# gudgud96/MR-MT3

Measured on AMD Instinct MI355X. Metric: train segments/sec (T5-small MT3Net, 256-frame mel, 1024-token target; log-mel + fwd + bwd + AdamW), higher is better.
Workload: dtype bf16; 1 GPU; BASELINE configs[1]: t5 bf16, 64 segments/GPU/step of 32768 samples @16kHz -> 256x512 mel, 1024-token targets, dropout 0.1 on, golden-recipe weights; segments_per_gpu=64, global_segments=64, parallelism=dp1

## Files before the change

include/mrmt3_hip.h:

```cpp
#ifndef MRMT3_HIP_H
#define MRMT3_HIP_H

#include <stddef.h>
#include <stdint.h>

#ifdef __cplusplus
extern "C" {
#endif

#define MRMT3_OK 0
#define MRMT3_ERR_INVALID_ARG 1
#define MRMT3_ERR_HIP 2
#define MRMT3_ERR_UNSUPPORTED 3
#define MRMT3_ERR_COMM 4

#define MRMT3_F32 0
#define MRMT3_BF16 1

int mrmt3_version(void);
const char* mrmt3_last_error(void);
void* mrmt3_host_alloc(size_t bytes);
void mrmt3_host_free(void* p);

#define MRMT3_CNT_GEMM_NT_TILE 0
// ... 167 lines not shown
                     int32_t* step_dev, float beta1, float beta2, float eps, float weight_decay,
                     float grad_scale, void* shadow_bf16, void* stream);
size_t mrmt3_grad_norm_workspace_elems(void);
int mrmt3_grad_norm(const float* g, size_t n, float grad_scale, float max_norm, int skip_nonfinite, float* ws,
                    size_t ws_elems, float* stat_dev, int32_t* skipped_dev, void* stream);
int mrmt3_adamw_step_clipped(float* p, const float* g, float* m, float* v, size_t n, const float* lr_dev,
                             int32_t* step_dev, float beta1, float beta2, float eps, float weight_decay,
                             float grad_scale, const float* stat_dev, float clip_value, void* shadow_bf16,
                             void* stream);
int mrmt3_counter_add(int32_t* ctr, int32_t delta, void* stream);
int mrmt3_transpose(const void* in, int in_dtype, void* out, int out_dtype, int rows, int cols,
                    void* stream);
int mrmt3_cast(const void* in, int in_dtype, void* out, int out_dtype, size_t n, void* stream);
int mrmt3_transpose_batched(const void* src_bf16, void* dst_bf16, const void* desc_table,
                            const int* tile_start, int n_mats, int total_tiles, void* stream);

typedef struct mrmt3_decoder mrmt3_decoder;
typedef struct {
  const void* embed;
  const float* pos;
  const void* lm_head;
  const float* final_ln;
  const float* const* ln_self;
  const void* const* w_qkv;
  const void* const* w_o_self;
  const float* const* ln_cross;
  const void* const* w_q_cross;
  const void* const* w_o_cross;
  const float* const* ln_ff;
  const void* const* w_wi;
// ... 52 lines not shown
```

mr-mt3_amd/csrc/api.hip:

```cpp
#include <stdarg.h>
#include <stdio.h>
#include <stdlib.h>

#include <atomic>
#include <mutex>

#include "common.h"

static thread_local char g_err[512] = "";

void mrmt3_set_error(const char* fmt, ...) {
  va_list ap;
  va_start(ap, fmt);
  vsnprintf(g_err, sizeof(g_err), fmt, ap);
  va_end(ap);
}

#ifdef MRMT3_DIAG
int mrmt3_diag_env(const char* name) {
  const char* e = getenv(name);
  const int v = e ? atoi(e) : 0;
  if (v != 0) {
    static std::atomic<unsigned> warned{0};
    const unsigned bit = 1u << ((unsigned char)name[6] & 31);
// ... 57 lines not shown
    strcpy(g_knob_over[g_knob_n_over++].name, name);
  }
  g_knob_over[i].value = value;
  for (MrKnob* k = g_knob_sites; k != nullptr; k = k->next)
    if (strcmp(k->name, name) == 0) __atomic_store_n(&k->state, 0, __ATOMIC_RELEASE);
  return MRMT3_OK;
}

extern "C" int mrmt3_reset_knobs(void) {
  std::lock_guard<std::mutex> lock(g_knob_mu);
  g_knob_n_over = 0;
  for (MrKnob* k = g_knob_sites; k != nullptr; k = k->next) __atomic_store_n(&k->state, 0, __ATOMIC_RELEASE);
  return MRMT3_OK;
}

extern "C" int mrmt3_version(void) { return 117;  }
extern "C" const char* mrmt3_last_error(void) { return g_err; }

int mrmt3_cu_count() {
  static int n = 0;
  if (n == 0) {
    int dev = 0;
    hipDeviceProp_t prop;
    if (hipGetDevice(&dev) == hipSuccess && hipGetDeviceProperties(&prop, dev) == hipSuccess) n = prop.multiProcessorCount;
    if (n <= 0) n = 256;
  }
  return n;
}

extern "C" void* mrmt3_host_alloc(size_t bytes) {
  void* p = nullptr;
// ... 118 lines not shown
```

mr-mt3_amd/csrc/rowops.hip:

```cpp
#include "common.h"

#pragma clang fp contract(off)

template <typename T> __device__ __forceinline__ void load4(const T* p, float v[4]);
template <> __device__ __forceinline__ void load4<float>(const float* p, float v[4]) {
  f32x4 t = *(const f32x4*)p;
  v[0] = t.x; v[1] = t.y; v[2] = t.z; v[3] = t.w;
}
template <> __device__ __forceinline__ void load4<bf16_t>(const bf16_t* p, float v[4]) {
  u32x2 t = *(const u32x2*)p;
  v[0] = __uint_as_float(t.x << 16); v[1] = __uint_as_float(t.x & 0xFFFF0000u);
  v[2] = __uint_as_float(t.y << 16); v[3] = __uint_as_float(t.y & 0xFFFF0000u);
}
template <typename T> __device__ __forceinline__ void store4(T* p, const float v[4]);
template <> __device__ __forceinline__ void store4<float>(float* p, const float v[4]) {
  *(f32x4*)p = f32x4{v[0], v[1], v[2], v[3]};
}
template <> __device__ __forceinline__ void store4<bf16_t>(bf16_t* p, const float v[4]) {
  *(u32x2*)p = u32x2{pack_bf2(v[0], v[1]), pack_bf2(v[2], v[3])};
}

template <typename T> __device__ __forceinline__ void load4_nt(const T* p, float v[4]);
template <> __device__ __forceinline__ void load4_nt<float>(const float* p, float v[4]) {
  const f32x4 t = __builtin_nontemporal_load((const f32x4*)p);
// ... 965 lines not shown
  for (int i = 0; i < TLP_REGS; ++i) se += expf(v[i] - mx);
  se = wave_sum(se);
  if (lane == 0) out[row] = (lp[t] - mx) - logf(se);
}

extern "C" int mrmt3_token_logprob(const float* logits, const int64_t* targets, float* out, int rows, int V,
                                   int ignore_index, void* stream) {
  MR_CHECK_ARG(logits && targets && out && rows > 0 && V > 0, "token_logprob: bad args");
  MR_CHECK_ARG(V <= 64 * TLP_REGS, "token_logprob: vocab %d exceeds the %d logits a wave keeps in registers", V, 64 * TLP_REGS);
  const dim3 grid((unsigned)ceil_div(rows, 4)), block(256);
  hipLaunchKernelGGL(token_logprob_kernel, grid, block, 0, (hipStream_t)stream, logits, targets, out, rows, V, ignore_index);
  MR_CHECK_LAUNCH("token_logprob");
  return MRMT3_OK;
}

__global__ void adamw_kernel(float* __restrict__ p, const float* __restrict__ g, float* __restrict__ m,
                             float* __restrict__ v, size_t n4, const float* __restrict__ lr_dev,
                             const int32_t* __restrict__ step_dev, float b1, float b2, float eps, float wd,
                             float gscale, bf16_t* __restrict__ shadow) {
  const float lr = lr_dev[0];
  const int step = step_dev[0] + 1;
  const double bc1 = 1.0 - pow((double)b1, (double)step);
  const double bc2 = 1.0 - pow((double)b2, (double)step);
  const float step_size = (float)((double)lr / bc1);
  const float bc2_sqrt = (float)sqrt(bc2);
  const float decay = 1.f - lr * wd;
  for (size_t i = (size_t)blockIdx.x * blockDim.x + threadIdx.x; i < n4; i += (size_t)gridDim.x * blockDim.x) {
    float pv[4], gv[4], mv[4], vv[4];
    load4<float>(p + i * 4, pv);
    load4<float>(g + i * 4, gv);
    load4<float>(m + i * 4, mv);
    load4<float>(v + i * 4, vv);
#pragma unroll
    for (int e = 0; e < 4; ++e) {
      const float gr = gv[e] * gscale;
      pv[e] *= decay;
      mv[e] = mv[e] + (gr - mv[e]) * (1.f - b1);
      vv[e] = vv[e] * b2 + (1.f - b2) * gr * gr;
      const float denom = sqrtf(vv[e]) / bc2_sqrt + eps;
      pv[e] -= step_size * (mv[e] / denom);
    }
    store4<float>(p + i * 4, pv);
    store4<float>(m + i * 4, mv);
    store4<float>(v + i * 4, vv);
    if (shadow) store4<bf16_t>(shadow + i * 4, pv);
  }
}
__global__ void step_inc_kernel(int32_t* step) { step[0] += 1; }

extern "C" int mrmt3_adamw_step(float* p, const float* g, float* m, float* v, size_t n, const float* lr_dev,
                                int32_t* step_dev, float beta1, float beta2, float eps, float weight_decay,
                                float grad_scale, void* shadow_bf16, void* stream) {
  MR_CHECK_ARG(p && g && m && v && lr_dev && step_dev && n % 4 == 0, "adamw_step: bad args");
  hipStream_t s = (hipStream_t)stream;
  hipLaunchKernelGGL(adamw_kernel, dim3(ew_blocks(n / 4)), dim3(256), 0, s, p, g, m, v, n / 4, lr_dev, step_dev,
                     beta1, beta2, eps, weight_decay, grad_scale, (bf16_t*)shadow_bf16);
  MR_CHECK_LAUNCH("adamw_step");
  hipLaunchKernelGGL(step_inc_kernel, dim3(1), dim3(1), 0, s, step_dev);
  MR_CHECK_LAUNCH("adamw_step inc");
  return MRMT3_OK;
}
// ... 85 lines not shown
  hipLaunchKernelGGL(grad_sumsq_kernel, dim3(GN_BLOCKS), dim3(256), 0, s, g, n / 4, (double*)ws);
  MR_CHECK_LAUNCH("grad_norm");
  hipLaunchKernelGGL(grad_norm_finish_kernel, dim3(1), dim3(256), 0, s, (const double*)ws, grad_scale, max_norm,
                     skip_nonfinite, stat_dev, skipped_dev);
  MR_CHECK_LAUNCH("grad_norm finish");
  return MRMT3_OK;
}

__global__ void adamw_clipped_kernel(float* __restrict__ p, const float* __restrict__ g, float* __restrict__ m,
                                     float* __restrict__ v, size_t n4, const float* __restrict__ lr_dev,
                                     const int32_t* __restrict__ step_dev, float b1, float b2, float eps, float wd,
                                     float gscale, const float* __restrict__ stat, float clip_value,
                                     bf16_t* __restrict__ shadow) {
  if (stat[2] != 0.f) return;
  const float coef = stat[1];
  const float lr = lr_dev[0];
  const int step = step_dev[0] + 1;
  const double bc1 = 1.0 - pow((double)b1, (double)step);
  const double bc2 = 1.0 - pow((double)b2, (double)step);
  const float step_size = (float)((double)lr / bc1);
  const float bc2_sqrt = (float)sqrt(bc2);
  const float decay = 1.f - lr * wd;
  for (size_t i = (size_t)blockIdx.x * blockDim.x + threadIdx.x; i < n4; i += (size_t)gridDim.x * blockDim.x) {
    float pv[4], gv[4], mv[4], vv[4];
    load4<float>(p + i * 4, pv);
    load4<float>(g + i * 4, gv);
    load4<float>(m + i * 4, mv);
    load4<float>(v + i * 4, vv);
#pragma unroll
    for (int e = 0; e < 4; ++e) {
      float gr = gv[e] * gscale * coef;
      if (clip_value > 0.f) gr = gr > clip_value ? clip_value : (gr < -clip_value ? -clip_value : gr);
      pv[e] *= decay;
      mv[e] = mv[e] + (gr - mv[e]) * (1.f - b1);
      vv[e] = vv[e] * b2 + (1.f - b2) * gr * gr;
      const float denom = sqrtf(vv[e]) / bc2_sqrt + eps;
      pv[e] -= step_size * (mv[e] / denom);
    }
    store4<float>(p + i * 4, pv);
    store4<float>(m + i * 4, mv);
    store4<float>(v + i * 4, vv);
    if (shadow) store4<bf16_t>(shadow + i * 4, pv);
  }
}

extern "C" int mrmt3_adamw_step_clipped(float* p, const float* g, float* m, float* v, size_t n, const float* lr_dev,
                                        int32_t* step_dev, float beta1, float beta2, float eps, float weight_decay,
                                        float grad_scale, const float* stat_dev, float clip_value, void* shadow_bf16,
                                        void* stream) {
  MR_CHECK_ARG(p && g && m && v && lr_dev && step_dev && stat_dev && n % 4 == 0, "adamw_step_clipped: bad args");
  MR_CHECK_ARG(clip_value >= 0.f, "adamw_step_clipped: clip_value = %g is negative (0: no clamp)", (double)clip_value);
  hipStream_t s = (hipStream_t)stream;
  hipLaunchKernelGGL(adamw_clipped_kernel, dim3(ew_blocks(n / 4)), dim3(256), 0, s, p, g, m, v, n / 4, lr_dev, step_dev,
                     beta1, beta2, eps, weight_decay, grad_scale, stat_dev, clip_value, (bf16_t*)shadow_bf16);
  MR_CHECK_LAUNCH("adamw_step_clipped");
  hipLaunchKernelGGL(step_inc_kernel, dim3(1), dim3(1), 0, s, step_dev);
  MR_CHECK_LAUNCH("adamw_step_clipped inc");
  return MRMT3_OK;
// ... 122 lines not shown
      if (r < d.rows) q[0] = v0;
      if (r + 1 < d.rows) q[1] = v1;
    }
  }
}

extern "C" int mrmt3_transpose_batched(const void* src_bf16, void* dst_bf16, const void* desc_table,
                                       const int* tile_start, int n_mats, int total_tiles, void* stream) {
  MR_CHECK_ARG(src_bf16 && dst_bf16 && desc_table && tile_start && n_mats > 0 && total_tiles > 0, "transpose_batched: bad args");
  hipLaunchKernelGGL(transpose_batched_kernel, dim3((unsigned)total_tiles), dim3(256), 0, (hipStream_t)stream,
                     (const bf16_t*)src_bf16, (bf16_t*)dst_bf16, (const TrDesc*)desc_table, tile_start, n_mats);
  MR_CHECK_LAUNCH("transpose_batched");
  return MRMT3_OK;
}

extern "C" int mrmt3_transpose(const void* in, int in_dtype, void* out, int out_dtype, int rows, int cols,
                               void* stream) {
  MR_CHECK_ARG(in && out && rows > 0 && cols > 0, "transpose: bad args");
  dim3 grid((unsigned)ceil_div(cols, 32), (unsigned)ceil_div(rows, 32)), block(256);
  hipStream_t s = (hipStream_t)stream;
  if (in_dtype == MRMT3_F32 && out_dtype == MRMT3_BF16)
    hipLaunchKernelGGL((transpose_kernel<float, bf16_t>), grid, block, 0, s, (const float*)in, (bf16_t*)out, rows, cols);
  else if (in_dtype == MRMT3_F32 && out_dtype == MRMT3_F32)
    hipLaunchKernelGGL((transpose_kernel<float, float>), grid, block, 0, s, (const float*)in, (float*)out, rows, cols);
  else if (in_dtype == MRMT3_BF16 && out_dtype == MRMT3_BF16)
    hipLaunchKernelGGL((transpose_kernel<bf16_t, bf16_t>), grid, block, 0, s, (const bf16_t*)in, (bf16_t*)out, rows, cols);
  else
    hipLaunchKernelGGL((transpose_kernel<bf16_t, float>), grid, block, 0, s, (const bf16_t*)in, (float*)out, rows, cols);
  MR_CHECK_LAUNCH("transpose");
  return MRMT3_OK;
// ... 2 lines not shown
```

mr-mt3_amd/mrmt3/engine.py:

```python
from __future__ import annotations

import os

import torch

from . import lib
from .params import FlatParams
from .synthetic import sinusoid_table


class Tape:

    def __init__(self):
        self.ops = []

    def push(self, **kw):
        self.ops.append(kw)

    def pop(self):
        return self.ops.pop()


class Engine:
    def __init__(self, cfg: dict, flat: FlatParams, variant: str = "t5", segmem_length: int = 64,
# ... 7 lines not shown
        self.eps = cfg["layer_norm_epsilon"]
        self.max_pos = max_pos
        self._pos = None
        self._stream_ctr = 0
        self.seed = 365
        self.step_dev = None
        self.y_dtype = compute_dtype
        self.overlap_wgrad = False
        self.res_grad_dtype = (torch.bfloat16 if compute_dtype == torch.bfloat16 and
                               os.environ.get("MRMT3_RES_GRAD", "bf16") == "bf16" else torch.float32)
        self.head_dtype = "bf16"
        self._wt32 = {}
        self.lo_sites = os.environ.get("MRMT3_ATTN_LO", "all")
        self.norm_dw = lib.NormDwBatch() if os.environ.get("MRMT3_NORM_DW_BATCH", "1") != "0" else None
        self.tn_group = lib.TnGroup() if os.environ.get("MRMT3_TN_GROUP", "1") != "0" else None
        self.fuse_rows = int(os.environ.get("MRMT3_FUSE_ROWS", "6")) if compute_dtype == torch.bfloat16 else 0
        self.fuse_normbwd_max_k = int(os.environ.get("MRMT3_FUSE_NORMBWD_MAXK", "1152"))

    def pos(self, device):
        if self._pos is None or self._pos.device != device:
            self._pos = sinusoid_table(self.max_pos, self.d).to(device).contiguous()
        return self._pos

    def _sid(self):
        self._stream_ctr += 1
        return self._stream_ctr

    def W(self, name):
        return self.flat.W(name, self.dt)

    def ln(self, key):
        return self.flat.master(key)

    def WT(self, name):
        if self.dt == torch.bfloat16:
            return self.flat.WT(name)
        t = self._wt32.get(name)
        if t is None:
            w = self.flat.W(name, torch.float32)
            t = torch.empty(w.shape[1], w.shape[0], device=w.device, dtype=torch.float32)
            lib.transpose(w, t)
            self._wt32[name] = t
        return t

    def wgrad(self, a, b, out):
        if a.dtype == torch.float32:
            return lib.gemm_tn_f32(a, b, out, accumulate=True)
        if self.tn_group is not None and self.tn_group.ok(a, b, out):
            return self.tn_group.add(a, b, out, accumulate=True)
        return lib.gemm_tn(a, b, out, accumulate=True)

    def _norm_bwd(self, *a, **kw):
        if self.dt == torch.bfloat16:
            return lib.add_rmsnorm_bwd(*a, defer=self.norm_dw, **kw)
        want_dy = kw.pop("want_dy", True)
        dx1, _ = lib.add_rmsnorm_bwd(*a, defer=self.norm_dw, want_dy=False, **kw)
        if not want_dy:
            return dx1, None
        p = kw.get("p", 0.0)
        if p <= 0.0:
            return dx1, dx1
        return dx1, lib.dropmask_cast(dx1, p=p, seed=kw.get("seed", 0), stream_id=kw.get("stream_y", 0),
                                      step=kw.get("step"), out_dtype=torch.float32)

# ... 359 lines not shown
        head_f32 = self.head_dtype == "f32" and tape is None and self.dt == torch.bfloat16
        dec = self.stack_fwd("decoder", x, B, Lx, cfg["num_decoder_layers"], True, enc=enc_cat, Le=Lc, p=p, tape=tape,
                             out_dtype=torch.float32 if head_f32 else None, pack=pack)
        if variant == "segmem_v1":
            dec = dec.view(B, Lx, d)[:, Ls:].contiguous().view(B * Ld, d)
        if tape is not None:
            tape.push(kind="head", dec=dec)
        if not want_logits:
            return dec, tape
        w_head = f.W("lm_head", torch.float32) if head_f32 else self.W("lm_head")
        logits = lib.gemm_nt(dec, w_head, out_dtype=torch.float32)
        if pack is not None:
            return logits, tape
        return logits.view(B, Ld, self.V), tape

    def backward(self, tape, dlogits, on_layer_done=None):
        f, cfg, d = self.flat, self.cfg, self.d
        variant, Ls = self.variant, self.segmem_length
        t = tape.pop()
        assert t["kind"] == "head"
        dl = dlogits.reshape(-1, self.V)
        if dl.dtype != self.dt:
            dl = self._act(dl)
        self.wgrad(dl, t["dec"], f.GW("lm_head"))
        d_dec = lib.gemm_nt(dl, self.WT("lm_head"), out_dtype=torch.float32)
        if on_layer_done is not None:
            on_layer_done("lm_head", 0)
        din = next(o for o in reversed(tape.ops) if o["kind"] == "dec_in")
        B, Le, Ld, Lx, Lc, Ls = din["B"], din["Le"], din["Ld"], din["Lx"], din["Lc"], din["Ls"]
        variant = din["variant"]
        if variant == "segmem_v1":
            full = torch.zeros(B, Lx, d, device=d_dec.device, dtype=torch.float32)
            full[:, Ls:] = d_dec.view(B, Ld, d)
# ... 36 lines not shown
```

mr-mt3_amd/mrmt3/lib.py:

```python
from __future__ import annotations

import ctypes as C
import os
import re
import subprocess

import torch

F32, BF16 = 0, 1
_HERE = os.path.dirname(os.path.abspath(__file__))
LIB_PATH = os.environ.get("MRMT3_TOOL_LIB") or os.path.join(_HERE, "libmrmt3_hip.so")
HEADER_PATH = os.path.join(os.path.dirname(os.path.dirname(_HERE)), "include", "mrmt3_hip.h")
CSRC_DIR = os.path.join(os.path.dirname(_HERE), "csrc")
_lib = None

vp = C.c_void_p


def _header_text(path: str) -> str:
    return re.sub(r"/\*.*?\*/", "", open(path).read(), flags=re.S)


def header_symbols(path: str = HEADER_PATH):
    return sorted(set(re.findall(r"\b(mrmt3_[a-z0-9_]+)\s*\(", _header_text(path))))
# ... 56 lines not shown
            "(no CPU fallback). Run `python __graft_entry__.py` / `make -C mr-mt3_amd/csrc` first.")
    lib = C.CDLL(LIB_PATH)
    for name, (res, args) in _SIGS.items():
        if os.environ.get("MRMT3_TOOL_LIB") and not hasattr(lib, name):
            continue
        fn = getattr(lib, name)
        fn.restype = res
        fn.argtypes = args
    if not os.environ.get("MRMT3_TOOL_LIB") and lib.mrmt3_version() < MIN_VERSION:
        raise RuntimeError(f"{LIB_PATH} is version {lib.mrmt3_version()}, this binding needs >= {MIN_VERSION}: "
                           "a stale build — run `make -C mr-mt3_amd/csrc`")
    _lib = lib
    return lib


MIN_VERSION = 117
COUNTER_NAMES = ("gemm_nt_tile", "gemm_nt8", "gemm_nt_geglu", "tn_group", "tn8", "tn_tile", "attn_fwd", "attn_bwd",
                 "attn_bwd_onepass", "attn_f32", "tn_f32", "gemm_nt_splitk", "gemm_nt_addnorm", "gemm_nt_normbwd",
                 "gemm_nt_geglubwd", "attn_fwd_varlen", "attn_bwd_varlen")


def set_knob(name: str, value: int):
    _check(load().mrmt3_set_knob(name.encode(), int(value)), "set_knob")


def reset_knobs():
    _check(load().mrmt3_reset_knobs(), "reset_knobs")


def dispatch_counts(reset: bool = False) -> dict:
    arr = (C.c_ulonglong * len(COUNTER_NAMES))()
# ... 787 lines not shown
    return out


def cast(src, out):
    _dev(src, out)
    _check(load().mrmt3_cast(_p(src), _dt(src), _p(out), _dt(out), src.numel(), _stream()), "cast")
    return out


def transpose_batched(src_flat, dst_flat, desc_table, tile_start, n_mats, total_tiles):
    _dev(src_flat, dst_flat, desc_table, tile_start)
    _check(load().mrmt3_transpose_batched(_p(src_flat), _p(dst_flat), _p(desc_table), _p(tile_start), n_mats,
                                          total_tiles, _stream()), "transpose_batched")


COMM_ID_BYTES = 128


class Comm:

    def __init__(self, uid: bytes, rank: int, world: int):
        assert len(uid) == COMM_ID_BYTES
        self.rank, self.world = rank, world
        self._h = vp()
        buf = C.create_string_buffer(uid, COMM_ID_BYTES)
        _check(load().mrmt3_comm_create(buf, rank, world, C.byref(self._h)), "comm_create")
        import weakref
        self._fin = weakref.finalize(self, Comm._destroy, self._h)

    @staticmethod
# ... 92 lines not shown
```

mr-mt3_amd/mrmt3/params.py:

```python
from __future__ import annotations

from collections import OrderedDict

import torch

from . import lib
from .synthetic import state_dict_shapes


class FlatParams:
    def __init__(self, cfg: dict, segmem_num_layers: int = 0, device="cpu"):
        self.cfg = cfg
        self.shapes = state_dict_shapes(cfg, segmem_num_layers)
        self.offsets: "OrderedDict[str, int]" = OrderedDict()
        off = 0
        n_dec = cfg["num_decoder_layers"]
        ckv = [f"decoder.block.{i}.layer.1.EncDecAttention.{n}.weight" for i in range(n_dec) for n in ("k", "v")]
        ckv_set = set(ckv)
        order = []
        for k in self.shapes:
            if k in ckv_set:
                continue
            if k == "decoder.block.0.layer.0.SelfAttention.q.weight":
                order.extend(ckv)
# ... 2 lines not shown
        for k in order:
            self.offsets[k] = off
            n = 1
            for s in self.shapes[k]:
                n *= s
            off += n
        self.numel = off
        assert off % 4 == 0
        self.P = torch.zeros(off, dtype=torch.float32, device=device)
        self.G = None
        self.M = None
        self.V = None
        self.S = None
        self.ST = None
        self._shadow_version = -1
        self.version_sources = ()
        self._build_groups(segmem_num_layers)

    def _build_groups(self, segmem_num_layers):
        cfg = self.cfg
        d, inner, dff = cfg["d_model"], cfg["d_kv"] * cfg["num_heads"], cfg["d_ff"]
        g: "OrderedDict[str, tuple]" = OrderedDict()

        def add(name, first_key, rows, cols):
            g[name] = (self.offsets[first_key], rows, cols)

        def stack(prefix, n, dec):
            for i in range(n):
                b = f"{prefix}.block.{i}.layer"
                add(f"{prefix}.{i}.qkv", f"{b}.0.SelfAttention.q.weight", 3 * inner, d)
# ... 81 lines not shown
        for t in self.version_sources:
            v += t._version
        return v

    def refresh_shadows(self, force=False, need_transposed=True):
        if not self.P.is_cuda:
            raise RuntimeError("bf16 shadows live on the GPU (no CPU fallback)")
        ver = self.master_version()
        have_t = self.ST is not None
        if not force and self.S is not None and ver == self._shadow_version and (have_t or not need_transposed):
            return
        if self.S is None or self.S.device != self.P.device:
            self.S = torch.empty(self.numel, dtype=torch.bfloat16, device=self.P.device)
        if force or ver != self._shadow_version or self._shadow_version < 0:
            lib.cast(self.P, self.S)
        if need_transposed:
            self.refresh_transposed()
        self._shadow_version = ver

    def refresh_transposed(self):
        import numpy as np
        if self.ST is None or self.ST.device != self.P.device:
            self.ST = torch.empty(self.t_numel, dtype=torch.bfloat16, device=self.P.device)
            self._tr_tab = None
        if getattr(self, "_tr_tab", None) is None:
            rec, starts, tot = [], [], 0
            for name, (o, r, c) in self.groups.items():
                if name not in self.t_offsets:
                    continue
                rec.append((o, self.t_offsets[name], r, c))
                starts.append(tot)
                tot += ((r + 63) // 64) * ((c + 63) // 64)
            tab = np.zeros(len(rec), dtype=[("src", "<i8"), ("dst", "<i8"), ("rows", "<i4"), ("cols", "<i4")])
            for i, t in enumerate(rec):
                tab[i] = t
            self._tr_tab = torch.from_numpy(tab.view(np.uint8).copy()).to(self.P.device)
            self._tr_start = torch.tensor(starts, dtype=torch.int32, device=self.P.device)
            self._tr_n, self._tr_tiles = len(rec), tot
        lib.transpose_batched(self.S, self.ST, self._tr_tab, self._tr_start, self._tr_n, self._tr_tiles)

    def adamw_step(self, lr_dev, step_dev, betas=(0.9, 0.999), eps=1e-8, weight_decay=0.01, grad_scale=1.0):
        self._optimizer_launch(lambda: lib.adamw_step(self.P, self.G, self.M, self.V, lr_dev, step_dev, betas[0], betas[1],
                                                      eps, weight_decay, grad_scale, shadow=self.S))

    def adamw_step_clipped(self, lr_dev, step_dev, stat_dev, betas=(0.9, 0.999), eps=1e-8, weight_decay=0.01, grad_scale=1.0,
                           clip_value=0.0):
        self._optimizer_launch(lambda: lib.adamw_step_clipped(self.P, self.G, self.M, self.V, lr_dev, step_dev, stat_dev,
                                                              betas[0], betas[1], eps, weight_decay, grad_scale, clip_value,
                                                              shadow=self.S))

    def _optimizer_launch(self, launch):
        self.ensure_adam()
        if self.S is None:
            self.refresh_shadows()
        launch()
        self.refresh_transposed()
        self._shadow_version = self.master_version()

    def load_numpy(self, weights: dict):
        for k, v in weights.items():
            self.master(k).copy_(torch.from_numpy(v).to(self.P.device))
```

mr-mt3_amd/mrmt3/trainer.py:

```python
from __future__ import annotations

import os

import torch
import torch.distributed as dist

from . import lib
from .ddp import GradBuckets


_RETIRED = []


def _retire(graph) -> None:
    import ctypes
    _RETIRED.append(graph)
    ctypes.pythonapi.Py_IncRef(ctypes.py_object(graph))


def _first_line(e) -> str:
    t = str(e)
    return t.splitlines()[0] if t else ""


# ... 52 lines not shown
        self.step_dev = torch.zeros(1, device=dev, dtype=torch.int32)
        self.host_step = 0
        self.world = dist.get_world_size() if dist.is_available() and dist.is_initialized() else 1
        cfg = model.cfg
        if grad_exchange_dtype is None and os.environ.get("MRMT3_GRAD_EXCHANGE", "f32") == "bf16":
            grad_exchange_dtype = torch.bfloat16
        layers_per_bucket = max(1, int(os.environ.get("MRMT3_DDP_LAYERS_PER_BUCKET", layers_per_bucket)))
        self.buckets = GradBuckets(self.flat, cfg["num_layers"], cfg["num_decoder_layers"],
                                   model.segmem_num_layers > 0, layers_per_bucket, exchange_dtype=grad_exchange_dtype)
        self.buckets.before_fire = model.engine.join_wgrad
        self.flat.ensure_grads()
        self.flat.ensure_adam()
        if self.world > 1:
            dist.broadcast(self.flat.P, src=0)
        self.last_loss = None
        self._clip_stat = self._skipped_dev = self._clip_ws = None
        if self.clip_on:
            self._clip_stat = torch.zeros(4, device=dev, dtype=torch.float32)
            self._skipped_dev = torch.zeros(1, device=dev, dtype=torch.int32)
            self._clip_ws = lib.grad_norm_workspace(dev)
        self.salt_dev = self.step_dev if n_acc == 1 else torch.zeros(1, device=dev, dtype=torch.int32)
        self.engine.step_dev = self.salt_dev
        self.use_graph = (os.environ.get("MRMT3_TRAIN_GRAPH", "1") != "0") if graph is None else bool(graph)
        self._collective_stream_checked = False
        self.graph_warmup = 2
        self._graphs = {}
        self._eager_seen = {}
        self._cap_stream = None
        self._cap_owner = None
        self.pack_graphs = max(1, int(os.environ.get("MRMT3_PACK_GRAPHS", "4")))
# ... 31 lines not shown
    def _step_body(self, inputs, labels, targets_prev, audio, cut=None, tcap=None, phase=None):
        eng, flat = self.engine, self.flat
        eng.reset_deferred()
        eng._stream_ctr = 0
        mel = self.mel_from_audio(inputs) if audio else inputs
        plan = self._pack_plan(labels, tcap)
        targets = labels.reshape(-1) if plan is None else plan.targets
        if eng.dt == torch.bfloat16:
            dec, tape = eng.forward(mel, labels, targets_prev, training=True, need_grad=True, want_logits=False, pack=plan)
            loss, dl = lib.lmhead_cross_entropy(dec, eng.W("lm_head"), targets, want_grad=True,
                                                grad_dtype=torch.bfloat16, weighted=self.weighted)
        else:
            logits, tape = eng.forward(mel, labels, targets_prev, training=True, need_grad=True, pack=plan)
            loss, dl = lib.cross_entropy(logits.reshape(-1, logits.shape[-1]), targets, want_grad=True,
                                         grad_dtype=torch.float32, weighted=self.weighted)
        if phase in (None, "first"):
            flat.G.zero_()
        self.buckets.reset()
        if phase in ("first", "middle"):
            eng.backward(tape, dl)
        elif cut is None:
            eng.backward(tape, dl, on_layer_done=self.buckets.on_layer_done)
            self.buckets.finish()
        else:
            sent = set()

            def layer_done(prefix, i):
                idx = [j for j in self.buckets.triggered_by(prefix, i) if j not in sent]
                if idx:
                    sent.update(idx)
                    eng.join_wgrad()
                    cut(idx)
            active = self.buckets.active
            eng.backward(tape, dl, on_layer_done=layer_done if active else None)
            cut([j for j in range(len(self.buckets.buckets)) if j not in sent] if active else [])
        if phase in (None, "last"):
            self._optimizer_tail()
        if self.accumulate > 1:
            lib.counter_add(self.salt_dev, 1)
        return loss

    def _optimizer_tail(self):
        scale = 1.0 / (self.world * self.accumulate)
        if not self.clip_on:
            self.flat.adamw_step(self.lr_dev, self.step_dev, self.betas, self.eps, self.wd, grad_scale=scale)
            return
        lib.grad_norm(self.flat.G, scale, self._max_norm, self.skip_nonfinite, self._clip_ws, self._clip_stat,
                      self._skipped_dev)
        self.flat.adamw_step_clipped(self.lr_dev, self.step_dev, self._clip_stat, self.betas, self.eps, self.wd,
                                     grad_scale=scale, clip_value=self._clip_value)

    @property
    def last_grad_norm(self):
        return None if self._clip_stat is None else self._clip_stat[0:1]

# ... 329 lines not shown
```

Measured before the change: 2740 segments/s.

## Fuse AdamW with transposed shadow refresh and skip zeroing of first-written grads

Adds one AdamW kernel that updates the master weights, writes the bf16 shadow, and writes the transposed bf16 shadow for each weight matrix through an LDS tile. This removes the separate batched-transpose pass over the shadow after every optimizer step. A span kernel handles the parameters that are not matrices, and an atomic arrival counter bumps the step counter once all blocks finish. The trainer also records which gradient regions backward writes directly on first write and zeroes only the complement, replacing the full G.zero_(). This adds complexity, including a runtime check that the recorded write coverage matches on later steps.

```diff
diff --git a/include/mrmt3_hip.h b/include/mrmt3_hip.h
--- a/include/mrmt3_hip.h
+++ b/include/mrmt3_hip.h
@@ -205,6 +205,14 @@
 int mrmt3_cast(const void* in, int in_dtype, void* out, int out_dtype, size_t n, void* stream);
 int mrmt3_transpose_batched(const void* src_bf16, void* dst_bf16, const void* desc_table,
                             const int* tile_start, int n_mats, int total_tiles, void* stream);
+int mrmt3_adamw_step_tr(float* p, const float* g, float* m, float* v, const float* lr_dev, int32_t* step_dev,
+                        float beta1, float beta2, float eps, float weight_decay, float grad_scale,
+                        const float* stat_dev, float clip_value, void* shadow_bf16, void* shadow_t_bf16,
+                        const void* desc_table, const int* tile_start, int n_mats, int total_tiles,
+                        const int64_t* span_off, const int* span_start4, int n_spans, int total_span4,
+                        int32_t* arrive_dev, void* stream);
+int mrmt3_zero_spans(float* base, const int64_t* span_off, const int* span_start4, int n_spans, int total4,
+                     void* stream);
 
 typedef struct mrmt3_decoder mrmt3_decoder;
 typedef struct {
diff --git a/mr-mt3_amd/csrc/api.hip b/mr-mt3_amd/csrc/api.hip
--- a/mr-mt3_amd/csrc/api.hip
+++ b/mr-mt3_amd/csrc/api.hip
@@ -95,7 +95,7 @@
   return MRMT3_OK;
 }
 
-extern "C" int mrmt3_version(void) { return 117;  }
+extern "C" int mrmt3_version(void) { return 118;  }
 extern "C" const char* mrmt3_last_error(void) { return g_err; }
 
 int mrmt3_cu_count() {
diff --git a/mr-mt3_amd/csrc/rowops.hip b/mr-mt3_amd/csrc/rowops.hip
--- a/mr-mt3_amd/csrc/rowops.hip
+++ b/mr-mt3_amd/csrc/rowops.hip
@@ -1003,37 +1003,55 @@
   return MRMT3_OK;
 }
 
+struct AdamwK { float step_size, bc2_sqrt, decay, b1, b2, eps; };
+__device__ __forceinline__ AdamwK adamw_consts(float lr, int step, float b1, float b2, float eps, float wd) {
+  const double bc1 = 1.0 - pow((double)b1, (double)step);
+  const double bc2 = 1.0 - pow((double)b2, (double)step);
+  AdamwK k;
+  k.step_size = (float)((double)lr / bc1);
+  k.bc2_sqrt = (float)sqrt(bc2);
+  k.decay = 1.f - lr * wd;
+  k.b1 = b1; k.b2 = b2; k.eps = eps;
+  return k;
+}
+__device__ __forceinline__ void adamw_elem(const AdamwK& k, float& p, float gr, float& m, float& v) {
+  p *= k.decay;
+  m = m + (gr - m) * (1.f - k.b1);
+  v = v * k.b2 + (1.f - k.b2) * gr * gr;
+  const float denom = sqrtf(v) / k.bc2_sqrt + k.eps;
+  p -= k.step_size * (m / denom);
+}
+template <bool CLIP>
+__device__ __forceinline__ float adamw_grad(float g, float gscale, float coef, float clip_value) {
+  if constexpr (!CLIP) return g * gscale;
+  float gr = g * gscale * coef;
+  if (clip_value > 0.f) gr = gr > clip_value ? clip_value : (gr < -clip_value ? -clip_value : gr);
+  return gr;
+}
+template <bool CLIP>
+__device__ __forceinline__ void adamw_update4(const AdamwK& k, float* __restrict__ p, const float* __restrict__ g,
+                                              float* __restrict__ m, float* __restrict__ v, size_t at, float gscale,
+                                              float coef, float clip_value, bf16_t* __restrict__ shadow) {
+  float pv[4], gv[4], mv[4], vv[4];
+  load4<float>(p + at, pv);
+  load4<float>(g + at, gv);
+  load4<float>(m + at, mv);
+  load4<float>(v + at, vv);
+#pragma unroll
+  for (int e = 0; e < 4; ++e) adamw_elem(k, pv[e], adamw_grad<CLIP>(gv[e], gscale, coef, clip_value), mv[e], vv[e]);
+  store4<float>(p + at, pv);
+  store4<float>(m + at, mv);
+  store4<float>(v + at, vv);
+  if (shadow) store4<bf16_t>(shadow + at, pv);
+}
+
 __global__ void adamw_kernel(float* __restrict__ p, const float* __restrict__ g, float* __restrict__ m,
                              float* __restrict__ v, size_t n4, const float* __restrict__ lr_dev,
                              const int32_t* __restrict__ step_dev, float b1, float b2, float eps, float wd,
                              float gscale, bf16_t* __restrict__ shadow) {
-  const float lr = lr_dev[0];
-  const int step = step_dev[0] + 1;
-  const double bc1 = 1.0 - pow((double)b1, (double)step);
-  const double bc2 = 1.0 - pow((double)b2, (double)step);
-  const float step_size = (float)((double)lr / bc1);
-  const float bc2_sqrt = (float)sqrt(bc2);
-  const float decay = 1.f - lr * wd;
-  for (size_t i = (size_t)blockIdx.x * blockDim.x + threadIdx.x; i < n4; i += (size_t)gridDim.x * blockDim.x) {
-    float pv[4], gv[4], mv[4], vv[4];
-    load4<float>(p + i * 4, pv);
-    load4<float>(g + i * 4, gv);
-    load4<float>(m + i * 4, mv);
-    load4<float>(v + i * 4, vv);
-#pragma unroll
-    for (int e = 0; e < 4; ++e) {
-      const float gr = gv[e] * gscale;
-      pv[e] *= decay;
-      mv[e] = mv[e] + (gr - mv[e]) * (1.f - b1);
-      vv[e] = vv[e] * b2 + (1.f - b2) * gr * gr;
-      const float denom = sqrtf(vv[e]) / bc2_sqrt + eps;
-      pv[e] -= step_size * (mv[e] / denom);
-    }
-    store4<float>(p + i * 4, pv);
-    store4<float>(m + i * 4, mv);
-    store4<float>(v + i * 4, vv);
-    if (shadow) store4<bf16_t>(shadow + i * 4, pv);
-  }
+  const AdamwK k = adamw_consts(lr_dev[0], step_dev[0] + 1, b1, b2, eps, wd);
+  for (size_t i = (size_t)blockIdx.x * blockDim.x + threadIdx.x; i < n4; i += (size_t)gridDim.x * blockDim.x)
+    adamw_update4<false>(k, p, g, m, v, i * 4, gscale, 1.f, 0.f, shadow);
 }
 __global__ void step_inc_kernel(int32_t* step) { step[0] += 1; }
 
@@ -1149,34 +1167,9 @@
                                      bf16_t* __restrict__ shadow) {
   if (stat[2] != 0.f) return;
   const float coef = stat[1];
-  const float lr = lr_dev[0];
-  const int step = step_dev[0] + 1;
-  const double bc1 = 1.0 - pow((double)b1, (double)step);
-  const double bc2 = 1.0 - pow((double)b2, (double)step);
-  const float step_size = (float)((double)lr / bc1);
-  const float bc2_sqrt = (float)sqrt(bc2);
-  const float decay = 1.f - lr * wd;
-  for (size_t i = (size_t)blockIdx.x * blockDim.x + threadIdx.x; i < n4; i += (size_t)gridDim.x * blockDim.x) {
-    float pv[4], gv[4], mv[4], vv[4];
-    load4<float>(p + i * 4, pv);
-    load4<float>(g + i * 4, gv);
-    load4<float>(m + i * 4, mv);
-    load4<float>(v + i * 4, vv);
-#pragma unroll
-    for (int e = 0; e < 4; ++e) {
-      float gr = gv[e] * gscale * coef;
-      if (clip_value > 0.f) gr = gr > clip_value ? clip_value : (gr < -clip_value ? -clip_value : gr);
-      pv[e] *= decay;
-      mv[e] = mv[e] + (gr - mv[e]) * (1.f - b1);
-      vv[e] = vv[e] * b2 + (1.f - b2) * gr * gr;
-      const float denom = sqrtf(vv[e]) / bc2_sqrt + eps;
-      pv[e] -= step_size * (mv[e] / denom);
-    }
-    store4<float>(p + i * 4, pv);
-    store4<float>(m + i * 4, mv);
-    store4<float>(v + i * 4, vv);
-    if (shadow) store4<bf16_t>(shadow + i * 4, pv);
-  }
+  const AdamwK k = adamw_consts(lr_dev[0], step_dev[0] + 1, b1, b2, eps, wd);
+  for (size_t i = (size_t)blockIdx.x * blockDim.x + threadIdx.x; i < n4; i += (size_t)gridDim.x * blockDim.x)
+    adamw_update4<true>(k, p, g, m, v, i * 4, gscale, coef, clip_value, shadow);
 }
 
 extern "C" int mrmt3_adamw_step_clipped(float* p, const float* g, float* m, float* v, size_t n, const float* lr_dev,
@@ -1329,6 +1322,168 @@
   return MRMT3_OK;
 }
 
+
+__device__ __forceinline__ int span_of(const int* __restrict__ start, int n, int i) {
+  int lo = 0, hi = n - 1;
+  while (lo < hi) {
+    const int mid = (lo + hi + 1) >> 1;
+    if (start[mid] <= i) lo = mid; else hi = mid - 1;
+  }
+  return lo;
+}
+
+template <bool CLIP>
+__global__ __launch_bounds__(256) void adamw_tr_kernel(float* __restrict__ p, const float* __restrict__ g,
+                                                       float* __restrict__ m, float* __restrict__ v,
+                                                       const float* __restrict__ lr_dev, int32_t* step_dev, float b1,
+                                                       float b2, float eps, float wd, float gscale,
+                                                       const float* __restrict__ stat, float clip_value,
+                                                       bf16_t* __restrict__ shadow, bf16_t* __restrict__ shadow_t,
+                                                       const TrDesc* __restrict__ tab, const int* __restrict__ tile_start,
+                                                       int n_mats, int total_tiles, int tile_blocks,
+                                                       const long long* __restrict__ span_off,
+                                                       const int* __restrict__ span_start4, int n_spans, int total_span4,
+                                                       int32_t* arrive) {
+  __shared__ __attribute__((aligned(16))) bf16_t tile[TRB][TRB + 2];
+  const int step0 = step_dev[0];
+  const bool skip = CLIP && stat[2] != 0.f;
+  if (!skip) {
+    const float coef = CLIP ? stat[1] : 1.f;
+    const AdamwK k = adamw_consts(lr_dev[0], step0 + 1, b1, b2, eps, wd);
+    if ((int)blockIdx.x < tile_blocks) {
+      unsigned* t32 = (unsigned*)&tile[0][0];
+      for (int t = blockIdx.x; t < total_tiles; t += tile_blocks) {
+        const int mi = span_of(tile_start, n_mats, t);
+        const TrDesc d = tab[mi];
+        const int local = t - tile_start[mi];
+        const int tiles_x = (d.cols + TRB - 1) / TRB;
+        const int bx = (local % tiles_x) * TRB, by = (local / tiles_x) * TRB;
+        const int r = threadIdx.x >> 4, c = (threadIdx.x & 15) * 4;
+        const bool col_in = bx + c < d.cols;
+        float pv[4][4], gv[4][4], mv[4][4], vv[4][4];
+#pragma unroll
+        for (int ps = 0; ps < 4; ++ps) {
+          const int rr = by + r + 16 * ps;
+          if (col_in && rr < d.rows) {
+            const size_t at = (size_t)d.src + (size_t)rr * d.cols + bx + c;
+            load4<float>(p + at, pv[ps]);
+            load4<float>(g + at, gv[ps]);
+            load4<float>(m + at, mv[ps]);
+            load4<float>(v + at, vv[ps]);
+          }
+        }
+#pragma unroll
+        for (int ps = 0; ps < 4; ++ps) {
+          const int rr = by + r + 16 * ps;
+          unsigned w0 = 0, w1 = 0;
+          if (col_in && rr < d.rows) {
+            const size_t at = (size_t)d.src + (size_t)rr * d.cols + bx + c;
+#pragma unroll
+            for (int e = 0; e < 4; ++e)
+              adamw_elem(k, pv[ps][e], adamw_grad<CLIP>(gv[ps][e], gscale, coef, clip_value), mv[ps][e], vv[ps][e]);
+            store4<float>(p + at, pv[ps]);
+            store4<float>(m + at, mv[ps]);
+            store4<float>(v + at, vv[ps]);
+            w0 = pack_bf2(pv[ps][0], pv[ps][1]);
+            w1 = pack_bf2(pv[ps][2], pv[ps][3]);
+            *(u32x2*)(shadow + at) = u32x2{w0, w1};
+          }
+          unsigned* q = t32 + (r + 16 * ps) * 33 + (c >> 1);
+          q[0] = w0; q[1] = w1;
+        }
+        __syncthreads();
+        if ((((d.rows | d.cols) & 7) == 0) && (((d.src | d.dst) & 7) == 0) && bx + TRB <= d.cols && by + TRB <= d.rows) {
+          const int r8 = threadIdx.x >> 3, c8 = threadIdx.x & 7;
+#pragma unroll
+          for (int hlf = 0; hlf < 2; ++hlf) {
+            const int oc = r8 + 32 * hlf;
+            unsigned w[4];
+#pragma unroll
+            for (int q = 0; q < 4; ++q)
+              w[q] = (unsigned)tile[c8 * 8 + 2 * q][oc] | ((unsigned)tile[c8 * 8 + 2 * q + 1][oc] << 16);
+            *(u32x4*)(shadow_t + d.dst + (size_t)(bx + oc) * d.rows + by + c8 * 8) = u32x4{w[0], w[1], w[2], w[3]};
+          }
+        } else {
+          const int tp = threadIdx.x & 31, ty = threadIdx.x >> 5;
+          const bool even = ((d.rows | d.cols) & 1) == 0 && ((d.src | d.dst) & 1) == 0;
+          for (int j = ty; j < TRB; j += 8) {
+            const int oc = bx + j, orow = by + 2 * tp;
+            if (oc >= d.cols) continue;
+            bf16_t* q = shadow_t + d.dst + (size_t)oc * d.rows + orow;
+            const bf16_t v0 = tile[2 * tp][j], v1 = tile[2 * tp + 1][j];
+            if (even && orow + 1 < d.rows) *(unsigned*)q = (unsigned)v0 | ((unsigned)v1 << 16);
+            else {
+              if (orow < d.rows) q[0] = v0;
+              if (orow + 1 < d.rows) q[1] = v1;
+            }
+          }
+        }
+        __syncthreads();
+      }
+    } else {
+      const int nb = (int)gridDim.x - tile_blocks;
+      for (int i = ((int)blockIdx.x - tile_blocks) * 256 + (int)threadIdx.x; i < total_span4; i += nb * 256) {
+        const int si = span_of(span_start4, n_spans, i);
+        adamw_update4<CLIP>(k, p, g, m, v, (size_t)span_off[si] + (size_t)(i - span_start4[si]) * 4, gscale, coef,
+                            clip_value, shadow);
+      }
+    }
+  }
+  asm volatile("s_waitcnt vmcnt(0)" ::: "memory");
+  __syncthreads();
+  if (threadIdx.x == 0 &&
+      __hip_atomic_fetch_add(arrive, 1, __ATOMIC_RELAXED, __HIP_MEMORY_SCOPE_AGENT) == (int)gridDim.x - 1) {
+    step_dev[0] = step0 + 1;
+    __hip_atomic_store(arrive, 0, __ATOMIC_RELAXED, __HIP_MEMORY_SCOPE_AGENT);
+  }
+}
+
+extern "C" int mrmt3_adamw_step_tr(float* p, const float* g, float* m, float* v, const float* lr_dev, int32_t* step_dev,
+                                   float beta1, float beta2, float eps, float weight_decay, float grad_scale,
+                                   const float* stat_dev, float clip_value, void* shadow_bf16, void* shadow_t_bf16,
+                                   const void* desc_table, const int* tile_start, int n_mats, int total_tiles,
+                                   const int64_t* span_off, const int* span_start4, int n_spans, int total_span4,
+                                   int32_t* arrive_dev, void* stream) {
+  MR_CHECK_ARG(p && g && m && v && lr_dev && step_dev && shadow_bf16 && shadow_t_bf16 && arrive_dev, "adamw_step_tr: null pointer");
+  MR_CHECK_ARG(desc_table && tile_start && n_mats > 0 && total_tiles > 0, "adamw_step_tr: no matrix table");
+  MR_CHECK_ARG(n_spans >= 0 && total_span4 >= 0 && (n_spans == 0) == (total_span4 == 0) && (n_spans == 0 || (span_off && span_start4)),
+               "adamw_step_tr: bad span table");
+  MR_CHECK_ARG(clip_value >= 0.f, "adamw_step_tr: clip_value = %g is negative (0: no clamp)", (double)clip_value);
+  const int tile_blocks = total_tiles < 4096 ? total_tiles : 4096;
+  const int span_blocks = n_spans ? ew_blocks((size_t)total_span4) : 0;
+  const dim3 grid((unsigned)(tile_blocks + span_blocks)), block(256);
+  hipStream_t s = (hipStream_t)stream;
+  if (stat_dev)
+    hipLaunchKernelGGL(adamw_tr_kernel<true>, grid, block, 0, s, p, g, m, v, lr_dev, step_dev, beta1, beta2, eps,
+                       weight_decay, grad_scale, stat_dev, clip_value, (bf16_t*)shadow_bf16, (bf16_t*)shadow_t_bf16,
+                       (const TrDesc*)desc_table, tile_start, n_mats, total_tiles, tile_blocks,
+                       (const long long*)span_off, span_start4, n_spans, total_span4, arrive_dev);
+  else
+    hipLaunchKernelGGL(adamw_tr_kernel<false>, grid, block, 0, s, p, g, m, v, lr_dev, step_dev, beta1, beta2, eps,
+                       weight_decay, grad_scale, stat_dev, clip_value, (bf16_t*)shadow_bf16, (bf16_t*)shadow_t_bf16,
+                       (const TrDesc*)desc_table, tile_start, n_mats, total_tiles, tile_blocks,
+                       (const long long*)span_off, span_start4, n_spans, total_span4, arrive_dev);
+  MR_CHECK_LAUNCH("adamw_step_tr");
+  return MRMT3_OK;
+}
+
+__global__ __launch_bounds__(256) void zero_spans_kernel(float* __restrict__ base, const long long* __restrict__ span_off,
+                                                         const int* __restrict__ span_start4, int n_spans, int total4) {
+  for (int i = (int)blockIdx.x * 256 + (int)threadIdx.x; i < total4; i += (int)gridDim.x * 256) {
+    const int si = span_of(span_start4, n_spans, i);
+    *(f32x4*)(base + (size_t)span_off[si] + (size_t)(i - span_start4[si]) * 4) = f32x4{0.f, 0.f, 0.f, 0.f};
+  }
+}
+
+extern "C" int mrmt3_zero_spans(float* base, const int64_t* span_off, const int* span_start4, int n_spans, int total4,
+                                void* stream) {
+  MR_CHECK_ARG(base && span_off && span_start4 && n_spans > 0 && total4 > 0 && ((uintptr_t)base & 15) == 0, "zero_spans: bad args");
+  hipLaunchKernelGGL(zero_spans_kernel, dim3(ew_blocks((size_t)total4)), dim3(256), 0, (hipStream_t)stream, base,
+                     (const long long*)span_off, span_start4, n_spans, total4);
+  MR_CHECK_LAUNCH("zero_spans");
+  return MRMT3_OK;
+}
+
 extern "C" int mrmt3_transpose(const void* in, int in_dtype, void* out, int out_dtype, int rows, int cols,
                                void* stream) {
   MR_CHECK_ARG(in && out && rows > 0 && cols > 0, "transpose: bad args");
diff --git a/mr-mt3_amd/mrmt3/engine.py b/mr-mt3_amd/mrmt3/engine.py
--- a/mr-mt3_amd/mrmt3/engine.py
+++ b/mr-mt3_amd/mrmt3/engine.py
@@ -45,6 +45,7 @@
         self.lo_sites = os.environ.get("MRMT3_ATTN_LO", "all")
         self.norm_dw = lib.NormDwBatch() if os.environ.get("MRMT3_NORM_DW_BATCH", "1") != "0" else None
         self.tn_group = lib.TnGroup() if os.environ.get("MRMT3_TN_GROUP", "1") != "0" else None
+        self.begin_wgrads(False)
         self.fuse_rows = int(os.environ.get("MRMT3_FUSE_ROWS", "6")) if compute_dtype == torch.bfloat16 else 0
         self.fuse_normbwd_max_k = int(os.environ.get("MRMT3_FUSE_NORMBWD_MAXK", "1152"))
 
@@ -74,11 +75,29 @@
             self._wt32[name] = t
         return t
 
+    def begin_wgrads(self, first_write: bool):
+        self.first_write = bool(first_write)
+        self._wg_touched = []
+        self.first_written = []
+
+    def _wg_touch(self, out):
+        lo = out.data_ptr()
+        hi = lo + ((out.shape[0] - 1) * out.stride(0) + out.shape[1]) * out.element_size()
+        seen = any(l < hi and lo < h for l, h in self._wg_touched)
+        self._wg_touched.append((lo, hi))
+        return seen
+
     def wgrad(self, a, b, out):
+        seen = self._wg_touch(out)
         if a.dtype == torch.float32:
             return lib.gemm_tn_f32(a, b, out, accumulate=True)
         if self.tn_group is not None and self.tn_group.ok(a, b, out):
-            return self.tn_group.add(a, b, out, accumulate=True)
+            first = self.first_write and not seen and out.is_contiguous()
+            if first:
+                self.first_written.append((out.data_ptr(), out.numel()))
+            return self.tn_group.add(a, b, out, accumulate=not first)
+        if seen and self.tn_group is not None:
+            self.tn_group.flush()
         return lib.gemm_tn(a, b, out, accumulate=True)
 
     def _norm_bwd(self, *a, **kw):
@@ -468,9 +487,10 @@
             return logits, tape
         return logits.view(B, Ld, self.V), tape
 
-    def backward(self, tape, dlogits, on_layer_done=None):
+    def backward(self, tape, dlogits, on_layer_done=None, first_write=False):
         f, cfg, d = self.flat, self.cfg, self.d
         variant, Ls = self.variant, self.segmem_length
+        self.begin_wgrads(first_write)
         t = tape.pop()
         assert t["kind"] == "head"
         dl = dlogits.reshape(-1, self.V)
diff --git a/mr-mt3_amd/mrmt3/lib.py b/mr-mt3_amd/mrmt3/lib.py
--- a/mr-mt3_amd/mrmt3/lib.py
+++ b/mr-mt3_amd/mrmt3/lib.py
@@ -94,7 +94,7 @@
     return lib
 
 
-MIN_VERSION = 117
+MIN_VERSION = 118
 COUNTER_NAMES = ("gemm_nt_tile", "gemm_nt8", "gemm_nt_geglu", "tn_group", "tn8", "tn_tile", "attn_fwd", "attn_bwd",
                  "attn_bwd_onepass", "attn_f32", "tn_f32", "gemm_nt_splitk", "gemm_nt_addnorm", "gemm_nt_normbwd",
                  "gemm_nt_geglubwd", "attn_fwd_varlen", "attn_bwd_varlen")
@@ -912,6 +912,77 @@
                                           total_tiles, _stream()), "transpose_batched")
 
 
+class TrTable:
+
+    def __init__(self, mats, device):
+        import numpy as np
+        self.mats = [tuple(int(x) for x in t) for t in mats]
+        tab = np.zeros(len(self.mats), dtype=[("src", "<i8"), ("dst", "<i8"), ("rows", "<i4"), ("cols", "<i4")])
+        starts, tot = [], 0
+        for i, (src, dst, r, c) in enumerate(self.mats):
+            tab[i] = (src, dst, r, c)
+            starts.append(tot)
+            tot += ((r + 63) // 64) * ((c + 63) // 64)
+        self.tab = torch.from_numpy(tab.view(np.uint8).copy()).to(device)
+        self.start = torch.tensor(starts, dtype=torch.int32, device=device)
+        self.n, self.tiles = len(self.mats), tot
+
+
+class SpanTable:
+
+    def __init__(self, spans, device):
+        self.spans = [(int(o), int(n)) for o, n in spans if n > 0]
+        if any(o % 4 or n % 4 for o, n in self.spans):
+            raise ValueError("SpanTable: offsets and lengths must be multiples of 4")
+        start4 = [0]
+        for _, n in self.spans:
+            start4.append(start4[-1] + n // 4)
+        if start4[-1] >= 2 ** 31:
+            raise ValueError("SpanTable: more than 2^31 float4s")
+        self.n, self.total4 = len(self.spans), start4[-1]
+        self.off = torch.tensor([o for o, _ in self.spans] or [0], dtype=torch.int64, device=device)
+        self.start4 = torch.tensor(start4, dtype=torch.int32, device=device)
+
+
+def complement_spans(covered, numel):
+    out, at = [], 0
+    for o, n in sorted(covered):
+        if o < at:
+            raise ValueError("complement_spans: overlapping spans")
+        if o > at:
+            out.append((at, o - at))
+        at = o + n
+    if at > numel:
+        raise ValueError("complement_spans: a span ends past the buffer")
+    if at < numel:
+        out.append((at, numel - at))
+    return out
+
+
+def adamw_step_tr(p, g, m, v, lr_dev, step_dev, shadow, shadow_t, tr, spans, arrive, stat=None, beta1=0.9, beta2=0.999,
+                  eps=1e-8, weight_decay=0.01, grad_scale=1.0, clip_value=0.0):
+    _dev(p, g, m, v, lr_dev, step_dev, shadow, shadow_t, tr.tab, tr.start, spans.off, spans.start4, arrive)
+    assert shadow.dtype == torch.bfloat16 and shadow_t.dtype == torch.bfloat16 and arrive.dtype == torch.int32
+    assert all(src % 4 == 0 and c % 4 == 0 for src, _, _, c in tr.mats), "matrix offsets / row lengths: multiples of 4"
+    if stat is not None:
+        _dev(stat)
+        assert stat.dtype == torch.float32 and stat.numel() >= 3
+    _check(load().mrmt3_adamw_step_tr(_p(p), _p(g), _p(m), _p(v), _p(lr_dev), _p(step_dev), beta1, beta2, eps,
+                                      weight_decay, grad_scale, _p(stat), float(clip_value), _p(shadow), _p(shadow_t),
+                                      _p(tr.tab), _p(tr.start), tr.n, tr.tiles, _p(spans.off) if spans.n else None,
+                                      _p(spans.start4) if spans.n else None, spans.n, spans.total4, _p(arrive),
+                                      _stream()), "adamw_step_tr")
+
+
+def zero_spans(buf, spans):
+    _dev(buf, spans.off, spans.start4)
+    assert buf.dtype == torch.float32 and buf.is_contiguous()
+    assert all(o + n <= buf.numel() for o, n in spans.spans)
+    if spans.n:
+        _check(load().mrmt3_zero_spans(_p(buf), _p(spans.off), _p(spans.start4), spans.n, spans.total4, _stream()),
+               "zero_spans")
+
+
 COMM_ID_BYTES = 128
 
 
diff --git a/mr-mt3_amd/mrmt3/params.py b/mr-mt3_amd/mrmt3/params.py
--- a/mr-mt3_amd/mrmt3/params.py
+++ b/mr-mt3_amd/mrmt3/params.py
@@ -40,6 +40,7 @@
         self.S = None
         self.ST = None
         self._shadow_version = -1
+        self._st_stale = True
         self.version_sources = ()
         self._build_groups(segmem_num_layers)
 
@@ -151,47 +152,56 @@
             self.S = torch.empty(self.numel, dtype=torch.bfloat16, device=self.P.device)
         if force or ver != self._shadow_version or self._shadow_version < 0:
             lib.cast(self.P, self.S)
+            self._st_stale = True
         if need_transposed:
             self.refresh_transposed()
         self._shadow_version = ver
 
-    def refresh_transposed(self):
-        import numpy as np
+    def _tr_tables(self):
         if self.ST is None or self.ST.device != self.P.device:
             self.ST = torch.empty(self.t_numel, dtype=torch.bfloat16, device=self.P.device)
-            self._tr_tab = None
-        if getattr(self, "_tr_tab", None) is None:
-            rec, starts, tot = [], [], 0
-            for name, (o, r, c) in self.groups.items():
-                if name not in self.t_offsets:
-                    continue
-                rec.append((o, self.t_offsets[name], r, c))
-                starts.append(tot)
-                tot += ((r + 63) // 64) * ((c + 63) // 64)
-            tab = np.zeros(len(rec), dtype=[("src", "<i8"), ("dst", "<i8"), ("rows", "<i4"), ("cols", "<i4")])
-            for i, t in enumerate(rec):
-                tab[i] = t
-            self._tr_tab = torch.from_numpy(tab.view(np.uint8).copy()).to(self.P.device)
-            self._tr_start = torch.tensor(starts, dtype=torch.int32, device=self.P.device)
-            self._tr_n, self._tr_tiles = len(rec), tot
-        lib.transpose_batched(self.S, self.ST, self._tr_tab, self._tr_start, self._tr_n, self._tr_tiles)
+            self._tr = None
+            self._st_stale = True
+        if getattr(self, "_tr", None) is None:
+            mats = [(o, self.t_offsets[name], r, c) for name, (o, r, c) in self.groups.items() if name in self.t_offsets]
+            self._tr = lib.TrTable(mats, self.P.device)
+            self._rest = None
+            rest = lib.complement_spans([(o, r * c) for o, _, r, c in mats], self.numel)
+            if all(o % 4 == 0 and c % 4 == 0 for o, _, _, c in mats) and all(o % 4 == 0 and n % 4 == 0 for o, n in rest):
+                self._rest = lib.SpanTable(rest, self.P.device)
+            self._arrive = torch.zeros(1, dtype=torch.int32, device=self.P.device)
+        return self._tr
+
+    def refresh_transposed(self):
+        tr = self._tr_tables()
+        lib.transpose_batched(self.S, self.ST, tr.tab, tr.start, tr.n, tr.tiles)
+        self._st_stale = False
 
     def adamw_step(self, lr_dev, step_dev, betas=(0.9, 0.999), eps=1e-8, weight_decay=0.01, grad_scale=1.0):
-        self._optimizer_launch(lambda: lib.adamw_step(self.P, self.G, self.M, self.V, lr_dev, step_dev, betas[0], betas[1],
-                                                      eps, weight_decay, grad_scale, shadow=self.S))
+        self._optimizer_launch(lr_dev, step_dev, None, betas, eps, weight_decay, grad_scale, 0.0)
 
     def adamw_step_clipped(self, lr_dev, step_dev, stat_dev, betas=(0.9, 0.999), eps=1e-8, weight_decay=0.01, grad_scale=1.0,
                            clip_value=0.0):
-        self._optimizer_launch(lambda: lib.adamw_step_clipped(self.P, self.G, self.M, self.V, lr_dev, step_dev, stat_dev,
-                                                              betas[0], betas[1], eps, weight_decay, grad_scale, clip_value,
-                                                              shadow=self.S))
-
-    def _optimizer_launch(self, launch):
+        self._optimizer_launch(lr_dev, step_dev, stat_dev, betas, eps, weight_decay, grad_scale, clip_value)
+
+    def _optimizer_launch(self, lr_dev, step_dev, stat_dev, betas, eps, weight_decay, grad_scale, clip_value):
         self.ensure_adam()
         if self.S is None:
             self.refresh_shadows()
-        launch()
-        self.refresh_transposed()
+        self._tr_tables()
+        if self._rest is None:
+            if stat_dev is None:
+                lib.adamw_step(self.P, self.G, self.M, self.V, lr_dev, step_dev, betas[0], betas[1], eps, weight_decay,
+                               grad_scale, shadow=self.S)
+            else:
+                lib.adamw_step_clipped(self.P, self.G, self.M, self.V, lr_dev, step_dev, stat_dev, betas[0], betas[1], eps,
+                                       weight_decay, grad_scale, clip_value, shadow=self.S)
+            self.refresh_transposed()
+        else:
+            if self._st_stale:
+                self.refresh_transposed()
+            lib.adamw_step_tr(self.P, self.G, self.M, self.V, lr_dev, step_dev, self.S, self.ST, self._tr, self._rest,
+                              self._arrive, stat_dev, betas[0], betas[1], eps, weight_decay, grad_scale, clip_value)
         self._shadow_version = self.master_version()
 
     def load_numpy(self, weights: dict):
diff --git a/mr-mt3_amd/mrmt3/trainer.py b/mr-mt3_amd/mrmt3/trainer.py
--- a/mr-mt3_amd/mrmt3/trainer.py
+++ b/mr-mt3_amd/mrmt3/trainer.py
@@ -90,6 +90,8 @@
         if self.world > 1:
             dist.broadcast(self.flat.P, src=0)
         self.last_loss = None
+        self.first_write = True
+        self._fw_cover = {}
         self._clip_stat = self._skipped_dev = self._clip_ws = None
         if self.clip_on:
             self._clip_stat = torch.zeros(4, device=dev, dtype=torch.float32)
@@ -151,13 +153,21 @@
             logits, tape = eng.forward(mel, labels, targets_prev, training=True, need_grad=True, pack=plan)
             loss, dl = lib.cross_entropy(logits.reshape(-1, logits.shape[-1]), targets, want_grad=True,
                                          grad_dtype=torch.float32, weighted=self.weighted)
-        if phase in (None, "first"):
-            flat.G.zero_()
+        zero_point = phase in (None, "first")
+        first_write = zero_point and self.first_write
+        cover_key = (tuple(mel.shape), tuple(labels.shape), None if targets_prev is None else tuple(targets_prev.shape),
+                     tcap, phase, cut is not None)
+        cover = self._fw_cover.get(cover_key) if first_write else None
+        if zero_point:
+            if cover is None:
+                flat.G.zero_()
+            else:
+                lib.zero_spans(flat.G, cover[1])
         self.buckets.reset()
         if phase in ("first", "middle"):
-            eng.backward(tape, dl)
+            eng.backward(tape, dl, first_write=first_write)
         elif cut is None:
-            eng.backward(tape, dl, on_layer_done=self.buckets.on_layer_done)
+            eng.backward(tape, dl, on_layer_done=self.buckets.on_layer_done, first_write=first_write)
             self.buckets.finish()
         else:
             sent = set()
@@ -169,13 +179,31 @@
                     eng.join_wgrad()
                     cut(idx)
             active = self.buckets.active
-            eng.backward(tape, dl, on_layer_done=layer_done if active else None)
+            eng.backward(tape, dl, on_layer_done=layer_done if active else None, first_write=first_write)
             cut([j for j in range(len(self.buckets.buckets)) if j not in sent] if active else [])
+        if first_write:
+            self._note_first_written(cover_key, cover)
         if phase in (None, "last"):
             self._optimizer_tail()
         if self.accumulate > 1:
             lib.counter_add(self.salt_dev, 1)
         return loss
+
+    def _note_first_written(self, key, cover):
+        base, esz = self.flat.G.data_ptr(), self.flat.G.element_size()
+        wrote = sorted(((p - base) // esz, n) for p, n in self.engine.first_written)
+        if cover is not None:
+            if wrote != cover[0]:
+                raise RuntimeError("this step stored other weight gradients than the step its zero spans were recorded "
+                                   "from: parts of the gradient buffer were neither zeroed nor written")
+            return
+        if torch.cuda.is_current_stream_capturing() or not wrote:
+            return
+        try:
+            rest = lib.SpanTable(lib.complement_spans(wrote, self.flat.numel), self.flat.G.device)
+        except ValueError:
+            return
+        self._fw_cover[key] = (wrote, rest)
 
     def _optimizer_tail(self):
         scale = 1.0 / (self.world * self.accumulate)
```

Measured after the change: 2747 segments/s (median of 6 runs). Within noise of the previous version (+0.3%).
